# cokwa/bitHTM

Measured on AMD Instinct MI355X. Metric: HTM timesteps/sec (SP + TM, learning on), 65536 cols x 32 cells, higher is better.
Workload: dtype u32 bit-packed / f64 + f32 permanences; 1 GPU; configs[2]: 65536 columns x 32 cells, SP + TM learning on, 1 MI355X; input_dim=1024, column_dim=65536, cell_dim=32, active_columns=1311, patterns=50, pretrain_steps=500, segments=96476, segment_slots=128, hip_graph=True, hip_graph_requested=True, pipelined=True, repetitions=15, streamed_calls=True

## Files before the change

bithtm_amd/build.py:

```python

import json
import os
import re
import subprocess
import sys

HERE = os.path.dirname(os.path.abspath(__file__))
CSRC = os.path.join(HERE, "csrc")
LIB = os.path.join(HERE, "libbithtm_hip.so")
RESOURCES = os.path.join(HERE, "libbithtm_hip.resources.json")
OWN_REPORTS = {"htm_knn.h": os.path.join(HERE, "libbithtm_hip.knn.resources.json")}
SOURCES = ["htm_engine.hip"]
HEADERS = ["htm_dev.h", "htm_sp_kernels.h", "htm_tm_kernels.h", "htm_pipeline.h", "htm_record.h", "htm_reset.h", "htm_decode.h", "htm_stack.h", "htm_forecast.h", "htm_noise.h", "htm_group.h", "htm_tm_feed.h", "htm_sp_run.h", "htm_fork.h", "htm_scalar.h", "htm_live.h", "htm_fields.h", "htm_likelihood.h", "htm_classifier.h", "htm_knn.h", "htm_rng.h", "htm_fexp.h",
           os.path.join("..", "..", "include", "bithtm_hip.h")]
FLAGS = ["--offload-arch=gfx950", "-O3", "-std=c++17", "-fPIC", "-shared", "-ffp-contract=off",
         "-fno-fast-math", "-Wall", "-Wno-unused-result", "-Wno-unused-value",
         "-Rpass-analysis=kernel-resource-usage"]


def _stale():
    if not os.path.exists(LIB) or not all(os.path.exists(r) for r in [RESOURCES] + list(OWN_REPORTS.values())):
        return True
    t = os.path.getmtime(LIB)
    deps = [os.path.join(CSRC, s) for s in SOURCES + HEADERS] + [os.path.abspath(__file__)]
    return any(os.path.getmtime(d) > t for d in deps)


def _kernel_resources(log):
    fields = {"VGPRs": "vgprs", "AGPRs": "agprs", "SGPRs": "sgprs", "ScratchSize [bytes/lane]": "scratch_bytes_per_lane",
              "Occupancy [waves/SIMD]": "occupancy", "LDS Size [bytes/block]": "lds_bytes"}
    out, cur = {}, None
    for line in log.splitlines():
        m = re.search(r"^(?:(\S+?):\d+:\d+: )?remark: +([^:]+): (\S+) \[-Rpass-analysis=kernel-resource-usage\]", line)
        if not m:
            continue
        key, val = m.group(2).strip(), m.group(3)
        if key == "Function Name":
            cur = out.setdefault(os.path.basename(m.group(1) or ""), {}).setdefault(val, {})
        elif cur is not None and key in fields:
            cur[fields[key]] = int(val)
    return out


def _without_remarks(log):
    out, pending, in_remark = [], [], False
    for line in log.splitlines():
        if "kernel-resource-usage" in line:
            pending, in_remark = [], True
        elif line.startswith("In file included from"):
            pending.append(line)
            in_remark = False
        elif in_remark and re.match(r"\s*\d*\s*\|", line):
            continue
        else:
            out += pending + [line]
            pending, in_remark = [], False
    return "\n".join(out)


def build(force=False, verbose=False):
    if not force and not _stale():
        return LIB
    hipcc = os.environ.get("HIPCC", "/opt/rocm/bin/hipcc")
    extra = os.environ.get("BITHTM_EXTRA_FLAGS", "").split()
    cmd = [hipcc] + FLAGS + extra + [os.path.join(CSRC, s) for s in SOURCES] + ["-o", LIB]
    if verbose:
        print(" ".join(cmd), file=sys.stderr)
    r = subprocess.run(cmd, stdout=subprocess.PIPE, stderr=subprocess.STDOUT, text=True)
    if r.returncode != 0:
        raise RuntimeError("hipcc failed:\n" + r.stdout)
    by_header = _kernel_resources(r.stdout)
    for header, path in OWN_REPORTS.items():
        with open(path, "w") as f:
            json.dump(by_header.pop(header, {}), f, indent=0, sort_keys=True)
    with open(RESOURCES, "w") as f:
        json.dump({k: v for kernels in by_header.values() for k, v in kernels.items()}, f, indent=0, sort_keys=True)
    if verbose:
        rest = _without_remarks(r.stdout)
        if rest.strip():
            print(rest, file=sys.stderr)
    return LIB


def kernel_resources(header=None):
    build()
    path = RESOURCES if header is None else OWN_REPORTS[header]
    if not os.path.exists(path):
        return None
    with open(path) as f:
        return json.load(f)


def all_kernel_resources():
    parts = [kernel_resources()] + [kernel_resources(h) for h in OWN_REPORTS]
    return None if any(p is None for p in parts) else {k: v for p in parts for k, v in p.items()}


if __name__ == "__main__":
    print(build(force="--force" in sys.argv, verbose=True))
```

bithtm_amd/csrc/htm_engine.hip:

```cpp

#include <hip/hip_runtime.h>
#include <hip/hip_ext.h>
#include <dlfcn.h>
#include <stdint.h>
#include <stdio.h>
#include <string.h>
#include <algorithm>
#include <cfloat>
#include <climits>
#include <cmath>
#include <chrono>
#include <map>
#include <memory>
#include <mutex>
#include <string>
#include <tuple>
#include <type_traits>
#include <vector>

#include "../../include/bithtm_hip.h"
#include "htm_fexp.h"
#include "htm_rng.h"

#include "htm_dev.h"
#include "htm_sp_kernels.h"
#include "htm_tm_kernels.h"
#include "htm_pipeline.h"
#include "htm_record.h"
#include "htm_reset.h"
#include "htm_decode.h"
#include "htm_stack.h"
#include "htm_forecast.h"
#include "htm_noise.h"
#include "htm_group.h"
#include "htm_tm_feed.h"
#include "htm_sp_run.h"
#include "htm_fork.h"
#include "htm_scalar.h"
#include "htm_live.h"
#include "htm_fields.h"
#include "htm_likelihood.h"
#include "htm_classifier.h"
#include "htm_knn.h"


struct ncclUniqueIdBytes { char internal[128]; };

static thread_local std::string g_create_error;
static int (*g_rccl_destroy)(void *) = nullptr;

struct Knobs {
    int graph_steps, eager_below;
    bool trace;
    uint32_t trace_until;
    int lean, lean2_classify, lean2_order, step_split, fuse_tm, shard_window, step_window, tail_rows, scan_large, scan_large_above, scan_dyn;
    int defer_tail, shared_scan, shared_members;
    int lean_overlap, lean_learn, lean_learn_large, lean_scan, lean_scan_large, scan_blocks, sel_launch_digits;
    int cand_d, cand_pairwise, cls_rows_max, win_offset, cand_zoom, cand_speculate, cand_take_all, poll_delay, cand_others;
};

struct Sizes {
    int G;
    int sp_blocks, sel_blocks, c256_blocks, s1024_blocks, scan_blocks, zero_blocks, cus;
    int lean_learn_blocks, lean_learn_blocks_large, lean_scan_blocks, lean_scan_blocks_large, lean_overlap_blocks, lean2_classify_blocks;
    int lean2_overlap_blocks;
    int lean_resident_large;
    bool emit_fits, emit_fits_open;
    bool emit_fits_lean;
    int sel_passes_fused, sel_passes_full;
};

struct RunModes {
    bool recording, resetting, decoding, feeding;
    bool capturing = false;
    bool operator<(const RunModes &o) const {
        return std::tie(recording, resetting, decoding, feeding, capturing) < std::tie(o.recording, o.resetting, o.decoding, o.feeding, o.capturing);
    }
};

struct RunGraphKey {
    int p; RunModes modes; int learning; bool sp_done, next_sp, next_front, lean; int spec; bool large, emit_fused, wmode;
    int span; const void *bank; int n_inputs;
    auto tie() const { return std::tie(p, modes, learning, sp_done, next_sp, next_front, lean, spec, large, emit_fused, wmode, span, bank, n_inputs); }
    bool operator<(const RunGraphKey &o) const { return tie() < o.tie(); }
};

struct ShardGraphKey {
    int p, learning; bool front_done, front_next; int span, ranks, n_inputs; std::vector<std::tuple<int, bool, bool>> per_rank; const void *bank;
    auto tie() const { return std::tie(p, learning, front_done, front_next, span, ranks, n_inputs, per_rank, bank); }
    bool operator<(const ShardGraphKey &o) const { return tie() < o.tie(); }
};

struct TmRunGraphKey {
    int p; RunModes modes; int learning, spec; bool large; int span; const void *lists; int n_rows, n;
    auto tie() const { return std::tie(p, modes, learning, spec, large, span, lists, n_rows, n); }
    bool operator<(const TmRunGraphKey &o) const { return tie() < o.tie(); }
};

struct SpRunGraphKey {
    int p, learning; bool recording, emit_fused; int wmode, span; const void *bank; int n_inputs;
    auto tie() const { return std::tie(p, learning, recording, emit_fused, wmode, span, bank, n_inputs); }
    bool operator<(const SpRunGraphKey &o) const { return tie() < o.tie(); }
};

struct htm_handle {
    htm_config cfg;
    Dev d;
    Knobs knob;
    Sizes sz;
// ... 322 lines not shown
    if (defer_tail) { h->tail_pending = true; h->tail_p = p; return; }
    if (fuse && (front_wmode >= 0 || n_tail_rows)) {
        const LearnScan ls = learn_scan(h, (size_t)SEL_BINS * 4);
        const int grid = ls.blocks() + (n_tail_rows ? n_tail_rows : h->sz.lean_overlap_blocks);
        const char *name = n_tail_rows ? "tm_learn+tm_scan+sp_learn" : "tm_learn+tm_scan+shard_overlap";
        LAUNCH_ON(h, h->stream, ls.lds, name, kt_learn_scan_tail[ls.slot], grid, 256, d, p, ls.n_learn, ls.n_scan, ls.spec, bank, n_inputs, h->sz.G, front_wmode, n_tail_rows);
        return;
    }
    enqueue_tm_tail(h, p);
    if (front_wmode >= 0)
        LAUNCH(h, "shard_overlap", k_shard_overlap, h->sz.sp_blocks, RB, d, bank, n_inputs, h->sz.G, p, front_wmode, 1);
}

struct StepPlan { bool sp_done, next_sp, next_front; };

static bool can_pipeline(const htm_handle *h) {
    return h->cfg.enable_sp && h->cfg.enable_tm && h->world == 1 && h->emit_fused_open && h->d.sel_passes == 2;
}

static bool can_lean(const htm_handle *h) {
    return h->knob.lean && can_pipeline(h) && bitmap_fits_lds(h->d) && h->sz.emit_fits_lean;
}

static decltype(&k_learn_scan_emit<1, 6>) const kt_lse_large[4] = {k_learn_scan_emit<1, 4, false>, k_learn_scan_emit<2, 4, false>,
                                                                   k_learn_scan_emit<4, 4, false>, k_learn_scan_emit<8, 4, false>};
static decltype(&k_learn_scan_emit<1, 6>) const kt_lse_tab[4] = {k_learn_scan_emit<1, 6, true>, k_learn_scan_emit<2, 6, true>,
                                                                 k_learn_scan_emit<4, 6, true>, k_learn_scan_emit<8, 6, true>};
static decltype(&k_learn_scan_emit<1, 6>) lse_kernel(const Dev &d, int form) {
    return (form == LSE_TAB ? kt_lse_tab : form == LSE_LARGE ? kt_lse_large : kt_lse_plain)[epl_slot(d)];
}

static int lse_form(const htm_handle *h) { return scan_pool_is_large(h) ? LSE_LARGE : lean_tab(h->d) ? LSE_TAB : LSE_PLAIN; }

static void launch_learn_scan_emit(htm_handle *h, int p, int n_emit) {
    Dev &d = h->d;
    const int epl = learn_epl(d);
    const size_t lds = std::max(std::max(learn_lds(epl, 256), lean_scan_lds(d)), sizeof(EmitShared));
    const bool large = scan_pool_is_large(h), dyn = large && h->knob.scan_dyn > 0;
    const int n_learn = dyn ? h->sz.lean_learn_blocks_large : h->sz.lean_learn_blocks;
    int n_scan = large ? h->sz.lean_scan_blocks_large : h->sz.lean_scan_blocks;
    if (dyn) n_scan = std::max(64, h->sz.lean_resident_large - n_emit - n_learn);
    const int grid = n_emit + n_learn + n_scan;
    if (large && !dyn) n_scan = -n_scan;
    const int spec = dyn ? 0 : scan_spec_blocks(h);
    const char *lse_name = large ? "tm_learn+tm_scan_large+sp_emit" : "tm_learn+tm_scan+sp_emit";
    LAUNCH_ON(h, h->stream, lds, lse_name, lse_kernel(d, lse_form(h)), grid, 256, d, p, n_emit, n_learn, n_scan, spec);
}

static int lean2_classify_blocks(const htm_handle *h, int learning) {
    if (!learning) return 0;
    return scan_pool_is_large(h) && !h->knob.lean2_classify ? std::max(h->sz.lean2_classify_blocks, 192) : h->sz.lean2_classify_blocks;
}

static void launch_act_mid_rows(htm_handle *h, const char *name, size_t lds, int p, int learning, const uint32_t *bank, int n_inputs, int n_overlap) {
    Dev &d = h->d;
    const int n_act = act_blocks(d), n_cls = lean2_classify_blocks(h, learning), n_rows = learning ? d.k : 0;
    const int n_duty = n_overlap ? 0 : h->sz.c256_blocks, n_clear = d.WPC * h->sz.c256_blocks;
    LAUNCH_ON(h, h->stream, lds, name, k_act_mid_rows, n_act + 1 + n_cls + n_rows + n_overlap + n_duty + n_clear + h->sz.zero_blocks, 256,
              d, p, d.k, n_act, learning, n_cls, bank, n_inputs, n_rows, h->sz.G, n_overlap, n_duty, n_clear, h->knob.lean2_order);
}

static void enqueue_lean(htm_handle *h, int p, int learning, const uint32_t *bank, int n_inputs, StepPlan plan) {
    Dev &d = h->d;
    if (h->knob.lean == 2) {
        launch_act_mid_rows(h, "tm_activate+tm_mid+sp_learn+sp_overlap", (size_t)SEL_BINS * 4, p, learning, bank, n_inputs,
                            plan.next_sp ? h->sz.lean2_overlap_blocks : 0);
    } else {
        const int n_act = act_blocks(d), n_rows = learning ? d.k : 0;
        const int n_cls = learning ? kClassifyBlocks : 0, n_ov = plan.next_sp ? h->sz.lean_overlap_blocks : 0;
        LAUNCH(h, "tm_activate+sp_learn", k_act_rows, n_act + n_rows + (1 + d.WPC) * h->sz.c256_blocks, 256, d, p, d.k, n_act, bank, n_inputs, n_rows, h->sz.c256_blocks);
        LAUNCH_ON(h, h->stream, (size_t)SEL_BINS * 4, "tm_mid+sp_overlap", k_mid_overlap, 1 + n_cls + n_ov + h->sz.zero_blocks, 256, d, p, d.k, 1, learning, n_cls,
                  bank, n_inputs, h->sz.G, n_ov);
    }
    launch_learn_scan_emit(h, p, plan.next_sp ? h->sz.c256_blocks : 0);
}

static decltype(&k_learn_overlap<1>) const kt_learn_overlap[4] = {k_learn_overlap<1>, k_learn_overlap<2>, k_learn_overlap<4>, k_learn_overlap<8>};
static decltype(&k_scan_sel<true, 1>) const kt_scan_sel[4] = {k_scan_sel<true, 1>, k_scan_sel<false, 1>, k_scan_sel<true, 6>, k_scan_sel<false, 6>};

static void enqueue_pipelined(htm_handle *h, int p, int learning, const uint32_t *bank, int n_inputs, StepPlan plan) {
    Dev &d = h->d;
    const int n_cls = learning ? kClassifyBlocks : 0;
    const int n_emit = plan.next_sp ? h->sz.c256_blocks : 0;
    LAUNCH_ON(h, h->stream, sizeof(EmitShared), "tm_activate+sp_emit", k_open_emit, n_emit + act_blocks(d), 256, d, p, n_emit, d.k);
    const int n_rows = (plan.next_sp && learning) ? d.k : 0, n_duty = plan.next_sp ? h->sz.c256_blocks : 0;
    LAUNCH(h, "tm_mid+sp_learn", k_mid_rows, 1 + n_cls + n_rows + n_duty + h->sz.zero_blocks, 256, d, p, d.k, 1, learning, n_cls, bank, n_inputs, n_rows, 1, n_duty);
    LAUNCH_ON(h, h->stream, std::max(learn_lds(learn_epl(d)), (size_t)SEL_BINS * 4), "tm_learn+sp_overlap", kt_learn_overlap[epl_slot(d)],
              kLearnBlocks + (plan.next_front ? h->sz.sp_blocks : 0), RB, d, p, kLearnBlocks, bank, n_inputs, h->sz.G, p, 2);
    const bool use_lds = bitmap_fits_lds(d), large = scan_pool_is_large(h);
    const int n_sel = plan.next_front ? 64 : 0, n_clear = plan.next_sp ? h->sz.c256_blocks : 0;
    LAUNCH_ON(h, h->stream, std::max(scan_lds(d, use_lds), sizeof(SelShared)), large ? "tm_scan_large+sp_select" : "tm_scan+sp_select",
              kt_scan_sel[scan_slot(large, use_lds)], h->sz.scan_blocks + n_sel + n_clear, 256, d, p, n_sel, n_clear, p, scan_spec_blocks(h));
}

static void enqueue_cold_start(htm_handle *h, const uint32_t *bank, int n_inputs, int learning, StepPlan plan) {
    Dev &d = h->d;
    const int p = (int)(h->step_host & 1);
    if (plan.sp_done || !plan.next_sp) return;
    const int wmode = step_wmode(h);
    if (can_lean(h)) {
        enqueue_sp_front(h, bank, n_inputs, p, wmode);
        enqueue_sp_back(h, bank, n_inputs, p, 1, 0, false, wmode);
        return;
    }
    enqueue_sp_front(h, bank, n_inputs, p, wmode);
    enqueue_sp_back(h, bank, n_inputs, p, 1, EMIT_DUTY | EMIT_CLEAR, learning != 0, wmode);
    LAUNCH(h, "sp_overlap", k_sp_overlap, h->sz.sp_blocks, RB, d, bank, n_inputs, h->sz.G, p, p ^ 1, 1, 0);
    LAUNCH(h, "sp_select", k_sel_pass, h->sz.sel_blocks, RB, d, 1, p ^ 1);
}

static int reset_blocks(const Dev &d) { return std::max(1, std::min(1024, (d.C * d.KP + 255) / 256)); }

static void enqueue_run_reset(htm_handle *h, RunModes m, int p) {
    if (m.resetting) LAUNCH(h, "tm_reset", k_tm_reset, reset_blocks(h->d), 256, h->d, p, h->d_reset, m.recording ? h->d_rec : nullptr, 0u);
}

static void enqueue_rest(htm_handle *h, RunModes m, int p, const uint32_t *bank, int n_inputs, int learning, StepPlan plan) {
    enqueue_run_reset(h, m, p);
    if ((plan.sp_done || plan.next_sp) && can_lean(h)) {
// ... 187 lines not shown
        rc |= dalloc(h, &h->d_cols_stage, k);
    }
    if (h->knob.trace) rc |= dalloc(h, &d.trace, (size_t)8 * 4096 * 2);
    return rc;
}

static const char *env_str(const char *name) { return getenv(name); }
static int env_int(const char *name, int dflt, int lo = INT_MIN, int hi = INT_MAX) {
    const char *e = env_str(name);
    return e ? std::max(lo, std::min(hi, atoi(e))) : dflt;
}
static int env_flag(const char *name, int dflt) {
    const char *e = env_str(name);
    return e ? atoi(e) != 0 : dflt;
}

static Knobs read_knobs() {
    Knobs k;
    k.graph_steps = env_int("BITHTM_GRAPH_STEPS", 16, 1, 256);
    k.eager_below = env_int("BITHTM_EAGER_BELOW", 64, 0);
    k.trace = env_str("BITHTM_TRACE") != nullptr;
    const char *until = env_str("BITHTM_TRACE_UNTIL");
    k.trace_until = until ? (uint32_t)strtoul(until, nullptr, 10) : 0xFFFFFFFFu;
    k.lean = env_int("BITHTM_LEAN", 2, 0, 2);
    k.lean2_classify = env_int("BITHTM_LEAN2_CLASSIFY", 0, 1);
    k.step_split = env_flag("BITHTM_STEP_SPLIT", 1);
    {
        const char *e = env_str("BITHTM_LEAN2_ORDER");
        const int o = e ? (int)strtol(e, nullptr, 16) : 0x0312;
        int seen = 0, pos[4] = {-1, -1, -1, -1};
        for (int i = 0; i < 4; ++i) { const int r = (o >> (4 * (3 - i))) & 15; if (r < 4) { seen |= 1 << r; pos[r] = i; } }
        k.lean2_order = (o >= 0 && o <= 0x3333 && seen == 15 && pos[0] < pos[1]) ? o : 0x0312;
    }
    k.fuse_tm = env_flag("BITHTM_FUSE_TM", 1);
    k.shard_window = env_flag("BITHTM_SHARD_WINDOW", 1);
    k.scan_large = env_int("BITHTM_SCAN_LARGE", -1);
    k.scan_large_above = env_int("BITHTM_SCAN_LARGE_ABOVE", 3 * 1536 * SCAN_SEGS, 0);
    k.step_window = env_flag("BITHTM_STEP_WINDOW", 1);
    k.tail_rows = env_flag("BITHTM_TAIL_ROWS", 1);
    k.scan_dyn = env_flag("BITHTM_SCAN_DYN", 1);
    k.defer_tail = env_flag("BITHTM_DEFER_TAIL", 1);
    k.shared_scan = env_flag("BITHTM_SHARED_SCAN", 0);
    k.shared_members = env_int("BITHTM_SHARED_SCAN_MEMBERS", 0, 0);
    k.lean_overlap = env_int("BITHTM_LEAN_OVERLAP", 0, 1);
    k.lean_learn = env_int("BITHTM_LEAN_LEARN", 0, 1);
    k.lean_learn_large = env_int("BITHTM_LEAN_LEARN_LARGE", 0, 1);
    k.lean_scan = env_int("BITHTM_LEAN_SCAN", 0, 1);
    k.lean_scan_large = env_int("BITHTM_LEAN_SCAN_LARGE", 0, 1);
    k.scan_blocks = env_int("BITHTM_SCAN_BLOCKS", 0, 1);
    k.sel_launch_digits = env_int("BITHTM_SEL_LAUNCH_DIGITS", -1, 0);
    k.cand_d = env_int("BITHTM_CAND_D", CAND_D, 0, CAND_D);
    k.cand_pairwise = env_int("BITHTM_CAND_PAIRWISE", CAND_PAIRWISE, 0);
    k.cls_rows_max = env_int("BITHTM_CLASSIFY_WORDS_ABOVE", -1, 0);
    k.win_offset = env_int("BITHTM_SEL_WINDOW_OFFSET", 0, 0);
    k.cand_zoom = env_int("BITHTM_CAND_ZOOM", -1);
    k.cand_speculate = env_flag("BITHTM_CAND_SPECULATE", 1);
    k.cand_take_all = env_flag("BITHTM_CAND_TAKE_ALL", 1);
    k.poll_delay = env_int("BITHTM_POLL_DELAY", 7, 0, 64);
    k.cand_others = env_int("BITHTM_CAND_OTHERS", CAND_OTHERS, 0, CAND_OTHERS);
    return k;
}

static void size_launches(htm_handle *h) {
    Dev &d = h->d;
    const Knobs &k = h->knob;
    Sizes &z = h->sz;
    z.G = 1;
    while (z.G < d.W4 && z.G < 64) z.G <<= 1;
    const int rows_per_block = (RB / 64) * 4 * (64 / z.G);
    z.sp_blocks = std::max(1, std::min((d.c1 - d.c0 + rows_per_block - 1) / rows_per_block, 256));
    z.sel_blocks = std::max(1, std::min((d.sel_hi - d.sel_lo + RB - 1) / RB, 128));
    z.c256_blocks = (d.sel_hi - d.sel_lo + 255) / 256;
    z.s1024_blocks = std::max(1, (d.Scap + 1023) / 1024);
    z.scan_blocks = std::max(1, std::min((d.Lcap + SCAN_SEGS - 1) / SCAN_SEGS, 2048));
    if (z.scan_blocks > 256) z.scan_blocks = (z.scan_blocks + 255) & ~255;
    z.zero_blocks = std::max(1, std::min((d.Lcap / 128 + 4095) / 4096, 1024));
    z.lean_overlap_blocks = k.lean_overlap ? k.lean_overlap : z.sp_blocks * (RB / 256);
    z.lean2_overlap_blocks = d.planes ? (d.c1 - d.c0 + 255) / 256 : z.lean_overlap_blocks;
    z.lean_learn_blocks = k.lean_learn ? k.lean_learn : 512;
    z.lean_learn_blocks_large = k.lean_learn_large ? k.lean_learn_large : k.lean_learn ? z.lean_learn_blocks : 768;
    z.lean_scan_blocks = k.lean_scan ? k.lean_scan : (z.scan_blocks > 512 ? std::max(256, (z.scan_blocks * 3 / 8 + 255) & ~255) : z.scan_blocks);
    z.lean_scan_blocks_large = k.lean_scan_large ? k.lean_scan_large : k.lean_scan ? z.lean_scan_blocks : z.scan_blocks;
    if (k.scan_blocks) z.scan_blocks = k.scan_blocks;
    hipDeviceProp_t prop;
    const bool have_prop = hipGetDeviceProperties(&prop, h->device) == hipSuccess;
    z.cus = have_prop ? prop.multiProcessorCount : 256;
    int B = 0;
    while ((1ll << B) <= (long long)d.I) ++B;
    const int informative = std::min(64, 64 - (29 - B) - KEY_SHIFT);
    d.sel_passes = std::max(1, std::min(SEL_MAX_PASSES, (informative + SEL_DIGIT - 1) / SEL_DIGIT));
    d.low_zero = 64 - informative;
    int per_cu_emit = 0, per_cu_open = 0;
    if (have_prop && hipOccupancyMaxActiveBlocksPerMultiprocessor(&per_cu_emit, (const void *)k_sp_emit, 256, 0) == hipSuccess &&
        hipOccupancyMaxActiveBlocksPerMultiprocessor(&per_cu_open, (const void *)k_open_emit, 256, sizeof(EmitShared)) == hipSuccess) {
        z.emit_fits = z.c256_blocks <= std::min(1024, per_cu_emit * z.cus);
        z.emit_fits_open = z.emit_fits && z.c256_blocks + act_blocks(d) <= std::min(1024, per_cu_open * z.cus);
        int per_cu_lean = 1 << 30;
        z.lean_resident_large = 1 << 30;
        const size_t lean_lds = std::max(std::max(learn_lds(learn_epl(d), 256), lean_scan_lds(d)), sizeof(EmitShared));
        bool asked = h->cfg.enable_tm && z.emit_fits && lean_lds <= 64 * 1024;
        for (int form = LSE_TAB; asked && form <= LSE_LARGE; ++form) {
            if (form == LSE_TAB && !lean_tab(d)) continue;
            int per_cu = 0;
            asked = hipOccupancyMaxActiveBlocksPerMultiprocessor(&per_cu, (const void *)lse_kernel(d, form), 256, lean_lds) == hipSuccess;
            per_cu_lean = std::min(per_cu_lean, per_cu);
            if (asked && form == LSE_LARGE) z.lean_resident_large = per_cu * z.cus;
        }
        z.emit_fits_lean = asked && z.c256_blocks <= std::min(1024, per_cu_lean * z.cus);
        if (z.lean_resident_large == (1 << 30)) z.lean_resident_large = 4 * z.cus;
    } else {
        (void)hipGetLastError();
        z.emit_fits = z.emit_fits_open = z.emit_fits_lean = false;
        z.lean_resident_large = 1024;
    }
    if (k.lean2_classify) {
        z.lean2_classify_blocks = k.lean2_classify;
    } else {
        int per_cu = 0, resident = 1536;
        if (have_prop && hipOccupancyMaxActiveBlocksPerMultiprocessor(&per_cu, (const void *)k_act_mid_rows, 256, (size_t)SEL_BINS * 4) == hipSuccess)
            resident = per_cu * z.cus;
        else
            (void)hipGetLastError();
        const int others = act_blocks(d) + z.lean_overlap_blocks + d.k + 1;
        const int room = (resident - others) & ~7;
        z.lean2_classify_blocks = room >= 128 ? std::min(kClassifyBlocks, room) : 32;
    }
    z.sel_passes_full = d.sel_passes;
    z.sel_passes_fused = std::min(d.sel_passes, 2);
    if (k.sel_launch_digits >= 0) z.sel_passes_fused = std::max(2, std::min(d.sel_passes, k.sel_launch_digits));
}

extern "C" int htm_create(const htm_config *cfg, htm_handle **out) {
    if (!cfg || !out) return fail_create(nullptr, "htm_create: null argument", HTM_ERR_ARGUMENT);
    if (cfg->struct_bytes != sizeof(htm_config)) return fail_create(nullptr, "htm_create: htm_config size mismatch (ABI)", HTM_ERR_ARGUMENT);
    if (cfg->column_dim < 1 || cfg->active_columns < 1 || cfg->active_columns > cfg->column_dim)
        return fail_create(nullptr, "htm_create: need 1 <= active_columns <= column_dim", HTM_ERR_ARGUMENT);
    if (cfg->enable_sp && cfg->input_dim < 1) return fail_create(nullptr, "htm_create: input_dim < 1", HTM_ERR_ARGUMENT);
    if (cfg->enable_tm) {
        if (cfg->cell_dim < 1 || cfg->cell_dim > 64) return fail_create(nullptr, "htm_create: cell_dim must be in 1..64", HTM_ERR_ARGUMENT);
        if (cfg->segment_slots < 64 || cfg->segment_slots > MAX_SLOTS || cfg->segment_slots % 64)
            return fail_create(nullptr, "htm_create: segment_slots must be a multiple of 64 in 64..512", HTM_ERR_ARGUMENT);
        if (cfg->segment_capacity < 1) return fail_create(nullptr, "htm_create: segment_capacity < 1", HTM_ERR_ARGUMENT);
        if (cfg->segment_sampling_synapses < 1 || cfg->segment_sampling_synapses > 64)
            return fail_create(nullptr, "htm_create: segment_sampling_synapses must be in 1..64", HTM_ERR_ARGUMENT);
        if (cfg->segment_activation_threshold < cfg->segment_matching_threshold)
            return fail_create(nullptr, "htm_create: activation threshold < matching threshold", HTM_ERR_ARGUMENT);
        if ((long long)cfg->column_dim * (cfg->cell_dim > 32 ? 64 : 32) > 0x7FFFFFFFLL) return fail_create(nullptr, "htm_create: column_dim too large", HTM_ERR_ARGUMENT);
    }
    if (!cfg->enable_sp && !cfg->enable_tm) return fail_create(nullptr, "htm_create: nothing enabled", HTM_ERR_ARGUMENT);
    const int world = cfg->shard_world > 1 ? cfg->shard_world : 1;
    if (world > 1) {
        if (!cfg->enable_sp || !cfg->enable_tm) return fail_create(nullptr, "htm_create: a sharded handle needs SP and TM", HTM_ERR_ARGUMENT);
        if (cfg->cell_dim > 32) return fail_create(nullptr, "htm_create: a sharded handle takes cell_dim up to 32 (the exchange record carries one 32-bit word per column)", HTM_ERR_ARGUMENT);
        if (world > 64) return fail_create(nullptr, "htm_create: at most 64 shards", HTM_ERR_ARGUMENT);
        if (cfg->shard_rank < 0 || cfg->shard_rank >= world) return fail_create(nullptr, "htm_create: shard_rank out of range", HTM_ERR_ARGUMENT);
        if (cfg->column_dim % (world * 64)) return fail_create(nullptr, "htm_create: column_dim must be a multiple of 64 * shard_world", HTM_ERR_ARGUMENT);
    }

    htm_handle *h = new htm_handle();
    h->cfg = *cfg;
    h->device = cfg->device;
    h->rank = world > 1 ? cfg->shard_rank : 0;
    h->world = world;
    h->knob = read_knobs();
    hipError_t e = hipSetDevice(cfg->device);
    if (e != hipSuccess) return fail_create(h, std::string("hipSetDevice: ") + hipGetErrorString(e), HTM_ERR_HIP);
    if (cfg->use_caller_stream) {
        h->stream = (hipStream_t)cfg->stream;
    } else {
        e = hipStreamCreateWithFlags(&h->stream, hipStreamNonBlocking);
        if (e != hipSuccess) return fail_create(h, std::string("hipStreamCreate: ") + hipGetErrorString(e), HTM_ERR_HIP);
        h->own_stream = true;
    }
// ... 3724 lines not shown
```

bithtm_amd/csrc/htm_tm_kernels.h:

```cpp
#ifndef BITHTM_HTM_TM_KERNELS_H
#define BITHTM_HTM_TM_KERNELS_H


__global__ __launch_bounds__(256) void k_tm_load_active(Dev d, int p, const int *cols, int n) {
    for (int c = blockIdx.x * 256 + threadIdx.x; c < d.C * d.WPC; c += gridDim.x * 256) {
        d.act[p][c] = 0;
        d.pred[p][c] = 0;
        d.win[p][c] = 0;
        if (c < n) d.active_cols[p][c] = cols[c];
        if (c < d.colwords) d.colbits[p][c] = 0;
    }
}

__global__ __launch_bounds__(256) void k_tm_activate(Dev d, int p, int n_active, int want_winner) {
    role_activate<false, true>(d, p, want_winner, blockIdx.x, n_active);
}

__global__ __launch_bounds__(256) void k_tm_ext_winners(Dev d, int p, const int *cols, const uint32_t *winw, const uint32_t *unacc, int n, int pass) {
    const int i = blockIdx.x * 256 + threadIdx.x;
    if (pass == 0) { for (int c = i; c < d.C * d.WPC; c += gridDim.x * 256) d.win[p][c] = 0; return; }
    if (i < n * d.WPC) {
        const int col = cols[i / d.WPC], wi = col * d.WPC + i % d.WPC;
        if (i % d.WPC == 0) d.active_cols[p][i / d.WPC] = col;
        d.actw_id[i] = wi;
// ... 157 lines not shown
            const u64 m0 = spread32((uint32_t)b0) | (spread32((uint32_t)b1) << 1);
            const u64 m1 = spread32((uint32_t)(b0 >> 32)) | (spread32((uint32_t)(b1 >> 32)) << 1);
            if (lane_id() == 0 && base < d.Ipad) {
                u64 *mw = (u64 *)&mrow[base >> 5];
                mw[0] = m0;
                mw[1] = m1;
            }
            plane_diff_store<16>(d, row, base >> 3, base < d.Ipad, m0, m1, old);
        } else {
            const u64 m0 = spread32((uint32_t)b0) | (spread32((uint32_t)b1) << 1);
            const u64 m1 = spread32((uint32_t)(b0 >> 32)) | (spread32((uint32_t)(b1 >> 32)) << 1);
            plane_diff_store_late<16>(d, mrow, row, i0, m0, m1);
            if (lane_id() == 0 && base < d.Ipad) {
                u64 *mw = (u64 *)&mrow[base >> 5];
                mw[0] = m0;
                mw[1] = m1;
            }
        }
        if (i0 == 0) ROW_STAMP(3); else ROW_STAMP(5);
    }
    if (OWN) {
        __shared__ int s_own[TPR / 64];
        own_cn = (int)wave_sum((uint32_t)own_cn);
        if (lane_id() == 0) s_own[t >> 6] = own_cn;
        __syncthreads();
        if (t == 0) {
            int cn = 0;
#pragma unroll
            for (int wv = 0; wv < TPR / 64; ++wv) cn += s_own[wv];
            const int sp = p ^ 1;
            float dc = duty0 * d.mom;
            dc = dc + d.dinc;
            d.duty[row] = dc;
            d.overlap[sp][row] = cn;
            const float f = htm_exp_f32(d.coef * dc);
            const double bo = (double)f * (double)cn;
            d.boosted[sp][row] = bo;
            const u64 key = select_key(bo);
            d.key[sp][row] = key;
            const uint32_t bin = win_bin(key, wbase);
            if (bin != 0u) {
                atomicAdd(d.hist0 + (size_t)sp * HIST0_PAR + (size_t)(ri & (HIST_REP - 1)) * SEL_BINS + bin, 1u);
                atomicAdd(d.hist0 + (size_t)sp * HIST0_PAR + HIST0_FINE + (size_t)(ri & (COARSE_REP - 1)) * COARSE_STRIDE + (bin >> 6), 1u);
            }
        }
    }
}

template <typename T>
__device__ __forceinline__ T ld_agent(const T *ptr, int same_launch) {
    return same_launch ? __hip_atomic_load(ptr, __ATOMIC_RELAXED, __HIP_MEMORY_SCOPE_AGENT) : *ptr;
}
struct NoWait { __device__ __forceinline__ void operator()() const {} };
template <int BS, typename Wait = NoWait>
__device__ __forceinline__ void role_mid(const Dev &d, int p, int n_active, int want_winner, int learning, int blk, int n_cls, int same_launch = 0,
                                         Wait wait = Wait()) {
    Counters *c = d.ctr;
    __shared__ int s_words[BS];
    __shared__ uint32_t s_bits[BS];
    __shared__ int s_nwords;
    if (blk > 0) {
        if (!learning || !c->has_distal) return;
        const int q = p ^ 1;
        const int n = d.world > 1 ? c->L : c->S;
        bool waited = false;
        auto wait_once = [&]() { if (!waited) { wait(); waited = true; } };
        auto gather = [&](int seg, bool &cand, bool &punish, int &cell) {
            const uint32_t info = d.seg_info[seg];
            cell = d.seg_cell[seg];
            const float jit = d.seg_jit[seg];
            const int cw = cell >> 5, cb = cell & 31, col = cell >> d.LK;
            const bool on_col = (d.colbits[p][col >> 5] >> (col & 31)) & 1u;
            const bool unpred = !((d.pred[q][cw] >> cb) & 1u);
            const bool best = fabsf(jit - __uint_as_float(d.cellmax[q][cell])) < d.eps;
            cand = ((info >> 31) || (unpred && best)) && (on_col || !same_launch);
            punish = d.punish ? (d.punish[cw] >> cb) & 1u : !on_col;
        };
        auto decide = [&](bool cand, int cell) {
            return cand && ((ld_agent(&d.win[p][cell >> 5], same_launch) >> (cell & 31)) & 1u);
        };
        if (n <= (d.cls_rows_max >= 0 ? d.cls_rows_max : (same_launch ? 2 : 8) * n_cls * BS)) {
            for (int i0 = (blk - 1) * BS; i0 < n; i0 += n_cls * BS) {
                const int seg = i0 + (int)threadIdx.x;
                bool cand = false, punish = false;
                int cell = 0;
                if (seg < n && ((d.match_bits[q][seg >> 5] >> (seg & 31)) & 1u)) gather(seg, cand, punish, cell);
                wait_once();
                const bool learn = decide(cand, cell);
                if (learn || punish) d.seg_nsyn[seg] |= (int)SEG_BUSY;
                const u64 ml = __ballot(learn), mp = __ballot(punish);
                const int n_l = __popcll(ml), n_p = __popcll(mp);
                if (n_l + n_p == 0) continue;
                int base = 0;
                if (lane_id() == 0) base = atomicAdd(&c->n_work[p], n_l + n_p);
                base = wave_read(base, 0);
                if (learn) {
                    const int pos = base + __popcll(ml & lanemask_lt());
                    if (pos < d.work_cap) d.work[pos] = (uint32_t)seg; else atomicOr(&c->error, 4);
                }
                if (punish) {
                    const int pos = base + n_l + __popcll(mp & lanemask_lt());
                    if (pos < d.work_cap) d.work[pos] = (uint32_t)seg | 0x80000000u; else atomicOr(&c->error, 4);
                }
            }
            return;
        }
        const int nwords = (n + 31) >> 5;
        const bool by_xcd = n_cls % 8 == 0 && n_cls >= 256;
        const int G8 = by_xcd ? n_cls / 8 : 1, x = (blk - 1) & 7, g = (blk - 1) >> 3;
        const int per_class = ((nwords + 255) >> 8) * 32;
        const int n_turns = by_xcd ? (per_class + G8 - 1) / G8 : (nwords + n_cls - 1) / n_cls;
        for (int t0 = 0; t0 < n_turns; t0 += BS) {
            if (threadIdx.x == 0) s_nwords = 0;
            __syncthreads();
            const int T = t0 + (int)threadIdx.x;
            int w;
            if (by_xcd) {
                const int u = T * G8 + g;
                w = ((x + 8 * (u >> 5)) << 5) + (u & 31);
            } else {
                w = (blk - 1) + n_cls * T;
            }
            const uint32_t word = (T < n_turns && w < nwords) ? d.match_bits[q][w] : 0u;
            if (word) {
                const int slot = atomicAdd(&s_nwords, 1);
                s_words[slot] = w;
                s_bits[slot] = word;
            }
            __syncthreads();
            const int listed = s_nwords;
            for (int i0 = 0; i0 < listed; i0 += BS / 32) {
                const int i = i0 + ((int)threadIdx.x >> 5);
                const bool on = i < listed && ((s_bits[min(i, BS - 1)] >> (threadIdx.x & 31)) & 1u);
                const int seg = on ? s_words[i] * 32 + (int)(threadIdx.x & 31) : 0;
                bool cand = false, punish = false;
                int cell = 0;
                if (on) gather(seg, cand, punish, cell);
                wait_once();
                const bool learn = decide(cand, cell);
                if (learn || punish) d.seg_nsyn[seg] |= (int)SEG_BUSY;
                const u64 ml = __ballot(learn), mp = __ballot(punish);
                const int n_l = __popcll(ml), n_p = __popcll(mp);
                if (n_l + n_p == 0) continue;
                int base = 0;
                if (lane_id() == 0) base = atomicAdd(&c->n_work[p], n_l + n_p);
                base = wave_read(base, 0);
                if (learn) {
                    const int pos = base + __popcll(ml & lanemask_lt());
                    if (pos < d.work_cap) d.work[pos] = (uint32_t)seg; else atomicOr(&c->error, 4);
                }
                if (punish) {
                    const int pos = base + n_l + __popcll(mp & lanemask_lt());
                    if (pos < d.work_cap) d.work[pos] = (uint32_t)seg | 0x80000000u; else atomicOr(&c->error, 4);
                }
            }
        }
        return;
    }
    __shared__ uint32_t s_wave[16];
    __shared__ uint32_t s_cells;
    __shared__ int s_nneed;
    if (threadIdx.x == 0) { s_cells = 0; s_nneed = 0; }
    const int S = c->S, nb = (S + 1023) >> 10;
    const uint32_t recyc_first = (int)threadIdx.x < nb ? (uint32_t)d.recyc_cnt[threadIdx.x] : 0u;
    uint32_t carry_w = 0, carry_u = 0, n_cells = 0;
    constexpr int LPT = 8;
    static_assert(LPT == 8, "the list pass loads 8 entries per thread");
    const int n_slots = n_active * d.WPC;
    const int nb2 = (nb + 1023) >> 10;
    const int cnt2_first = ((int)threadIdx.x < 256 && (int)threadIdx.x < nb2) ? d.recyc_cnt2[threadIdx.x] : 0;
    const int prev_has_winner = c->has_winner[p ^ 1], prev_n_win = c->n_win[p ^ 1];
    const int has_distal_early = same_launch ? c->has_distal : 0;
    wait();
    for (int base = 0; base < n_slots; base += LPT * BS) {
        const int i0 = base + LPT * (int)threadIdx.x;
        uint32_t ww[LPT], uw[LPT];
        int a[LPT];
        uint32_t vsum = 0;
        u64 ac = 0;
        if (i0 < n_slots && same_launch) {
#pragma unroll
            for (int j = 0; j < LPT; j += 2) {
                const u64 av = __hip_atomic_load((const u64 *)(d.actw_id + i0 + j), __ATOMIC_RELAXED, __HIP_MEMORY_SCOPE_AGENT);
                const u64 wv = __hip_atomic_load((const u64 *)(d.winw_idx + i0 + j), __ATOMIC_RELAXED, __HIP_MEMORY_SCOPE_AGENT);
                const u64 uv = __hip_atomic_load((const u64 *)(d.unacc_word + i0 + j), __ATOMIC_RELAXED, __HIP_MEMORY_SCOPE_AGENT);
                a[j] = (int)(uint32_t)av; a[j + 1] = (int)(uint32_t)(av >> 32);
                ww[j] = (uint32_t)wv; ww[j + 1] = (uint32_t)(wv >> 32);
                uw[j] = (uint32_t)uv; uw[j + 1] = (uint32_t)(uv >> 32);
            }
            ac = __hip_atomic_load((const u64 *)(d.actcnt + i0), __ATOMIC_RELAXED, __HIP_MEMORY_SCOPE_AGENT);
        } else if (i0 < n_slots) {
            const int4 a0 = *(const int4 *)(d.actw_id + i0), a1 = *(const int4 *)(d.actw_id + i0 + 4);
            const uint4 w0 = *(const uint4 *)(d.winw_idx + i0), w1 = *(const uint4 *)(d.winw_idx + i0 + 4);
// ... 1042 lines not shown
```

Baseline: 43610 timesteps/s.

## Add handover kernel that builds winner and unaccounted lists in block0 with LDS staging

Adds a specialised variant of the fused activate/mid/rows kernel in which block 0 of the mid role compacts the winner and unaccounted-cell lists itself, then immediately binds recycled and new segments. The unaccounted list is staged in dynamic LDS up to a configurable cap, and scalar pointers are pinned to SGPRs. It also adds an option to prefetch seg_nsyn during gather so the busy mark is a plain store rather than a read-modify-write. The aim is to cut global round-trips and extra kernel phases on the per-step critical path, at the cost of more LDS per block and a possibly lower resident-block count, which the sizing now takes as the minimum over both kernels.

```diff
diff --git a/bithtm_amd/build.py b/bithtm_amd/build.py
--- a/bithtm_amd/build.py
+++ b/bithtm_amd/build.py
@@ -10,8 +10,9 @@
 LIB = os.path.join(HERE, "libbithtm_hip.so")
 RESOURCES = os.path.join(HERE, "libbithtm_hip.resources.json")
 OWN_REPORTS = {"htm_knn.h": os.path.join(HERE, "libbithtm_hip.knn.resources.json")}
+LATER_REPORTS = {"htm_handover.h": os.path.join(HERE, "libbithtm_hip.handover.resources.json")}
 SOURCES = ["htm_engine.hip"]
-HEADERS = ["htm_dev.h", "htm_sp_kernels.h", "htm_tm_kernels.h", "htm_pipeline.h", "htm_record.h", "htm_reset.h", "htm_decode.h", "htm_stack.h", "htm_forecast.h", "htm_noise.h", "htm_group.h", "htm_tm_feed.h", "htm_sp_run.h", "htm_fork.h", "htm_scalar.h", "htm_live.h", "htm_fields.h", "htm_likelihood.h", "htm_classifier.h", "htm_knn.h", "htm_rng.h", "htm_fexp.h",
+HEADERS = ["htm_dev.h", "htm_sp_kernels.h", "htm_tm_kernels.h", "htm_pipeline.h", "htm_record.h", "htm_reset.h", "htm_decode.h", "htm_stack.h", "htm_forecast.h", "htm_noise.h", "htm_group.h", "htm_tm_feed.h", "htm_sp_run.h", "htm_fork.h", "htm_scalar.h", "htm_live.h", "htm_fields.h", "htm_likelihood.h", "htm_classifier.h", "htm_knn.h", "htm_handover.h", "htm_rng.h", "htm_fexp.h",
            os.path.join("..", "..", "include", "bithtm_hip.h")]
 FLAGS = ["--offload-arch=gfx950", "-O3", "-std=c++17", "-fPIC", "-shared", "-ffp-contract=off",
          "-fno-fast-math", "-Wall", "-Wno-unused-result", "-Wno-unused-value",
@@ -19,7 +20,7 @@
 
 
 def _stale():
-    if not os.path.exists(LIB) or not all(os.path.exists(r) for r in [RESOURCES] + list(OWN_REPORTS.values())):
+    if not os.path.exists(LIB) or not all(os.path.exists(r) for r in [RESOURCES] + list(OWN_REPORTS.values()) + list(LATER_REPORTS.values())):
         return True
     t = os.path.getmtime(LIB)
     deps = [os.path.join(CSRC, s) for s in SOURCES + HEADERS] + [os.path.abspath(__file__)]
@@ -70,7 +71,7 @@
     if r.returncode != 0:
         raise RuntimeError("hipcc failed:\n" + r.stdout)
     by_header = _kernel_resources(r.stdout)
-    for header, path in OWN_REPORTS.items():
+    for header, path in list(OWN_REPORTS.items()) + list(LATER_REPORTS.items()):
         with open(path, "w") as f:
             json.dump(by_header.pop(header, {}), f, indent=0, sort_keys=True)
     with open(RESOURCES, "w") as f:
@@ -84,7 +85,7 @@
 
 def kernel_resources(header=None):
     build()
-    path = RESOURCES if header is None else OWN_REPORTS[header]
+    path = RESOURCES if header is None else OWN_REPORTS[header] if header in OWN_REPORTS else LATER_REPORTS[header]
     if not os.path.exists(path):
         return None
     with open(path) as f:
@@ -96,5 +97,10 @@
     return None if any(p is None for p in parts) else {k: v for p in parts for k, v in p.items()}
 
 
+def every_kernel_resources():
+    parts = [all_kernel_resources()] + [kernel_resources(h) for h in LATER_REPORTS]
+    return None if any(p is None for p in parts) else {k: v for p in parts for k, v in p.items()}
+
+
 if __name__ == "__main__":
     print(build(force="--force" in sys.argv, verbose=True))
diff --git a/bithtm_amd/csrc/htm_engine.hip b/bithtm_amd/csrc/htm_engine.hip
--- a/bithtm_amd/csrc/htm_engine.hip
+++ b/bithtm_amd/csrc/htm_engine.hip
@@ -42,6 +42,7 @@
 #include "htm_likelihood.h"
 #include "htm_classifier.h"
 #include "htm_knn.h"
+#include "htm_handover.h"
 
 
 struct ncclUniqueIdBytes { char internal[128]; };
@@ -55,6 +56,7 @@
     uint32_t trace_until;
     int lean, lean2_classify, lean2_order, step_split, fuse_tm, shard_window, step_window, tail_rows, scan_large, scan_large_above, scan_dyn;
     int defer_tail, shared_scan, shared_members;
+    int handover_cap;
     int lean_overlap, lean_learn, lean_learn_large, lean_scan, lean_scan_large, scan_blocks, sel_launch_digits;
     int cand_d, cand_pairwise, cls_rows_max, win_offset, cand_zoom, cand_speculate, cand_take_all, poll_delay, cand_others;
 };
@@ -483,19 +485,25 @@
     return scan_pool_is_large(h) && !h->knob.lean2_classify ? std::max(h->sz.lean2_classify_blocks, 192) : h->sz.lean2_classify_blocks;
 }
 
-static void launch_act_mid_rows(htm_handle *h, const char *name, size_t lds, int p, int learning, const uint32_t *bank, int n_inputs, int n_overlap) {
+static void launch_act_mid_rows(htm_handle *h, const char *name, size_t lds, int p, int learning, const uint32_t *bank, int n_inputs, int n_overlap,
+                                bool handover = false) {
     Dev &d = h->d;
     const int n_act = act_blocks(d), n_cls = lean2_classify_blocks(h, learning), n_rows = learning ? d.k : 0;
     const int n_duty = n_overlap ? 0 : h->sz.c256_blocks, n_clear = d.WPC * h->sz.c256_blocks;
-    LAUNCH_ON(h, h->stream, lds, name, k_act_mid_rows, n_act + 1 + n_cls + n_rows + n_overlap + n_duty + n_clear + h->sz.zero_blocks, 256,
-              d, p, d.k, n_act, learning, n_cls, bank, n_inputs, n_rows, h->sz.G, n_overlap, n_duty, n_clear, h->knob.lean2_order);
+    const int grid = n_act + 1 + n_cls + n_rows + n_overlap + n_duty + n_clear + h->sz.zero_blocks;
+    if (handover)
+        LAUNCH_ON(h, h->stream, std::max(lds, (size_t)SEL_BINS * 4), name, k_first_handover, grid, 256,
+                  d, p, d.k, n_act, learning, n_cls, bank, n_inputs, n_rows, h->sz.G, n_overlap, n_duty, n_clear, h->knob.lean2_order, h->knob.handover_cap);
+    else
+        LAUNCH_ON(h, h->stream, lds, name, k_act_mid_rows, grid, 256,
+                  d, p, d.k, n_act, learning, n_cls, bank, n_inputs, n_rows, h->sz.G, n_overlap, n_duty, n_clear, h->knob.lean2_order);
 }
 
 static void enqueue_lean(htm_handle *h, int p, int learning, const uint32_t *bank, int n_inputs, StepPlan plan) {
     Dev &d = h->d;
     if (h->knob.lean == 2) {
         launch_act_mid_rows(h, "tm_activate+tm_mid+sp_learn+sp_overlap", (size_t)SEL_BINS * 4, p, learning, bank, n_inputs,
-                            plan.next_sp ? h->sz.lean2_overlap_blocks : 0);
+                            plan.next_sp ? h->sz.lean2_overlap_blocks : 0, true);
     } else {
         const int n_act = act_blocks(d), n_rows = learning ? d.k : 0;
         const int n_cls = learning ? kClassifyBlocks : 0, n_ov = plan.next_sp ? h->sz.lean_overlap_blocks : 0;
@@ -789,6 +797,7 @@
     k.cand_d = env_int("BITHTM_CAND_D", CAND_D, 0, CAND_D);
     k.cand_pairwise = env_int("BITHTM_CAND_PAIRWISE", CAND_PAIRWISE, 0);
     k.cls_rows_max = env_int("BITHTM_CLASSIFY_WORDS_ABOVE", -1, 0);
+    k.handover_cap = env_int("BITHTM_HANDOVER_LDS_CAP", HANDOVER_LIST_MAX, 0, HANDOVER_LIST_MAX);
     k.win_offset = env_int("BITHTM_SEL_WINDOW_OFFSET", 0, 0);
     k.cand_zoom = env_int("BITHTM_CAND_ZOOM", -1);
     k.cand_speculate = env_flag("BITHTM_CAND_SPECULATE", 1);
@@ -854,8 +863,10 @@
         z.lean2_classify_blocks = k.lean2_classify;
     } else {
         int per_cu = 0, resident = 1536;
-        if (have_prop && hipOccupancyMaxActiveBlocksPerMultiprocessor(&per_cu, (const void *)k_act_mid_rows, 256, (size_t)SEL_BINS * 4) == hipSuccess)
-            resident = per_cu * z.cus;
+        int per_cu_run = 0;
+        if (have_prop && hipOccupancyMaxActiveBlocksPerMultiprocessor(&per_cu, (const void *)k_act_mid_rows, 256, (size_t)SEL_BINS * 4) == hipSuccess &&
+            hipOccupancyMaxActiveBlocksPerMultiprocessor(&per_cu_run, (const void *)k_first_handover, 256, (size_t)SEL_BINS * 4) == hipSuccess)
+            resident = std::min(per_cu, per_cu_run) * z.cus;
         else
             (void)hipGetLastError();
         const int others = act_blocks(d) + z.lean_overlap_blocks + d.k + 1;
diff --git a/bithtm_amd/csrc/htm_handover.h b/bithtm_amd/csrc/htm_handover.h
--- /dev/null
+++ b/bithtm_amd/csrc/htm_handover.h
@@ -0,0 +1,262 @@
+#ifndef BITHTM_HANDOVER_H
+#define BITHTM_HANDOVER_H
+
+#define HANDOVER_NEED 128
+#define HANDOVER_LIST_MAX (SEL_BINS - 2 * HANDOVER_NEED - 256)
+static_assert(HANDOVER_LIST_MAX >= 1024, "the dynamic LDS of the launch (SEL_BINS words) holds the list, the needed blocks and the counts");
+
+#ifdef BITHTM_HANDOVER_STAMPS
+#define HSTAMP(i, v) do { if (d.trace && threadIdx.x == 0 && d.ctr->step[p] < d.trace_until) d.trace[(size_t)(3 + 4 * p) * 8192 + (i)] = (v); } while (0)
+#else
+#define HSTAMP(i, v) do { } while (0)
+#endif
+
+template <typename Wait>
+__device__ __forceinline__ void role_handover_block0(const Dev &d, int p, int n_active, int learning, int list_cap, uint32_t *dyn, Wait wait) {
+    constexpr int BS = 256, LPT = 8;
+    Counters *c = d.ctr;
+    int *s_un = (int *)dyn, *s_need = (int *)dyn + HANDOVER_LIST_MAX, *s_cnt2 = s_need + 2 * HANDOVER_NEED;
+    __shared__ uint32_t s_wave[16];
+    __shared__ uint32_t s_cells;
+    __shared__ int s_nneed;
+    if (threadIdx.x == 0) { s_cells = 0; s_nneed = 0; }
+    const int S = c->S, nb = (S + 1023) >> 10;
+    const uint32_t recyc_first = (int)threadIdx.x < nb ? (uint32_t)d.recyc_cnt[threadIdx.x] : 0u;
+    int n_slots = n_active * d.WPC;
+    const int nb2 = (nb + 1023) >> 10;
+    const int cnt2_first = (int)threadIdx.x < nb2 ? d.recyc_cnt2[threadIdx.x] : 0;
+    const int prev_has_winner = c->has_winner[p ^ 1], prev_n_win = c->n_win[p ^ 1];
+    const int has_distal = c->has_distal;
+    typedef __attribute__((address_space(1))) int gint;
+    typedef __attribute__((address_space(1))) const u64 gu64c;
+    gu64c *actw_id = (gu64c *)d.actw_id, *winw_idx = (gu64c *)d.winw_idx, *unacc_word = (gu64c *)d.unacc_word, *actcnt = (gu64c *)d.actcnt;
+    gint *winners = (gint *)d.winners[p], *unacc_list = (gint *)d.unacc_list, *seg_nsyn = (gint *)d.seg_nsyn, *seg_cell = (gint *)d.seg_cell;
+    typedef __attribute__((address_space(1))) Counters gctr;
+    gctr *ctr = (gctr *)c;
+    int match_thr = d.match_thr, Scap = d.Scap;
+#ifndef BITHTM_HANDOVER_NO_PIN
+    asm volatile("" : "+s"(actw_id), "+s"(winw_idx), "+s"(unacc_word), "+s"(actcnt), "+s"(winners), "+s"(unacc_list), "+s"(seg_nsyn), "+s"(seg_cell),
+                      "+s"(match_thr), "+s"(Scap), "+s"(ctr), "+s"(n_slots));
+#endif
+    c = (Counters *)ctr;
+    HSTAMP(0, wall_clock64());
+    wait();
+    HSTAMP(1, wall_clock64());
+    uint32_t carry_w = 0, carry_u = 0, n_cells = 0;
+    uint32_t ww[LPT];
+    int a[LPT];
+    uint32_t run_w = 0;
+    for (int base = 0; base < n_slots; base += LPT * BS) {
+        const int i0 = base + LPT * (int)threadIdx.x;
+        uint32_t uw[LPT];
+        uint32_t vsum = 0;
+        u64 ac = 0;
+        if (i0 < n_slots) {
+#pragma unroll
+            for (int j = 0; j < LPT; j += 2) {
+                const u64 av = __hip_atomic_load(actw_id + ((i0 + j) >> 1), __ATOMIC_RELAXED, __HIP_MEMORY_SCOPE_AGENT);
+                const u64 wv = __hip_atomic_load(winw_idx + ((i0 + j) >> 1), __ATOMIC_RELAXED, __HIP_MEMORY_SCOPE_AGENT);
+                const u64 uv = __hip_atomic_load(unacc_word + ((i0 + j) >> 1), __ATOMIC_RELAXED, __HIP_MEMORY_SCOPE_AGENT);
+                a[j] = (int)(uint32_t)av; a[j + 1] = (int)(uint32_t)(av >> 32);
+                ww[j] = (uint32_t)wv; ww[j + 1] = (uint32_t)(wv >> 32);
+                uw[j] = (uint32_t)uv; uw[j + 1] = (uint32_t)(uv >> 32);
+            }
+            ac = __hip_atomic_load(actcnt + (i0 >> 3), __ATOMIC_RELAXED, __HIP_MEMORY_SCOPE_AGENT);
+#pragma unroll
+            for (int j = 0; j < LPT; ++j) {
+                const bool ok = i0 + j < n_slots;
+                if (!ok) { ww[j] = 0; uw[j] = 0; }
+                n_cells += ok ? (uint32_t)((ac >> (8 * j)) & 0xFFu) : 0u;
+            }
+        } else {
+#pragma unroll
+            for (int j = 0; j < LPT; ++j) { a[j] = 0; ww[j] = 0; uw[j] = 0; }
+        }
+#pragma unroll
+        for (int j = 0; j < LPT; ++j) vsum += (uint32_t)__popc(ww[j]) | ((uint32_t)__popc(uw[j]) << 16);
+        uint32_t total;
+        const uint32_t run = block_excl_scan<BS, true>(vsum, s_wave, total);
+        run_w = carry_w + (run & 0xFFFFu);
+        int pu = (int)(carry_u + (run >> 16));
+#pragma unroll
+        for (int j = 0; j < LPT; ++j) {
+            uint32_t u1 = uw[j];
+            while (u1) {
+                const int b = __ffs(u1) - 1;
+                u1 &= u1 - 1;
+                if (pu < list_cap) s_un[pu] = a[j] * 32 + b; else unacc_list[pu] = a[j] * 32 + b;
+                ++pu;
+            }
+        }
+        if (base + LPT * BS < n_slots) {
+            int pw = (int)run_w;
+#pragma unroll
+            for (int j = 0; j < LPT; ++j) {
+                uint32_t w1 = ww[j];
+                while (w1) { const int b = __ffs(w1) - 1; w1 &= w1 - 1; winners[pw++] = a[j] * 32 + b; }
+            }
+        }
+        carry_w += total & 0xFFFFu;
+        carry_u += total >> 16;
+    }
+    n_cells = wave_sum(n_cells);
+    if (lane_id() == 0) atomicAdd(&s_cells, n_cells);
+    const int n_un = (learning && has_distal) ? (int)carry_u : 0;
+    auto finish = [&](int n_r, int n_new, bool bound) {
+        int pw = (int)run_w;
+#pragma unroll
+        for (int j = 0; j < LPT; ++j) {
+            uint32_t w1 = ww[j];
+            while (w1) { const int b = __ffs(w1) - 1; w1 &= w1 - 1; winners[pw++] = a[j] * 32 + b; }
+        }
+        for (int i = threadIdx.x; i < min((int)carry_u, list_cap); i += BS) unacc_list[i] = s_un[i];
+        HSTAMP(8, wall_clock64());
+        if (threadIdx.x == 0) {
+            c->n_win[p] = (int)carry_w;
+            c->has_winner[p] = 1;
+            c->n_un = n_un;
+            c->n_active_cells = (int)s_cells;
+            c->n_bind[p] = bound ? n_r + n_new : 0;
+            if (bound) {
+                c->n_recycled = n_r;
+                c->n_new = n_new;
+                c->S_old = S;
+                c->S = S + n_new;
+            }
+        }
+    };
+    lds_barrier();
+    HSTAMP(2, wall_clock64());
+    HSTAMP(6, (unsigned long long)n_un);
+    if (n_un == 0) { finish(0, 0, false); return; }
+    uint32_t carry = 0;
+    for (int r0 = 0; r0 < nb2 && carry < (uint32_t)n_un; r0 += 256) {
+        lds_barrier();
+        s_cnt2[threadIdx.x] = r0 == 0 ? cnt2_first : (r0 + (int)threadIdx.x < nb2 ? d.recyc_cnt2[r0 + threadIdx.x] : 0);
+        lds_barrier();
+        for (int r = r0; r < min(r0 + 256, nb2) && carry < (uint32_t)n_un; ++r) {
+            if (s_cnt2[r - r0] == 0) continue;
+            for (int base = r << 10; base < min(nb, (r + 1) << 10); base += BS) {
+                const int b = base + threadIdx.x;
+                const uint32_t v = base == 0 ? recyc_first : ((b < nb && b < ((r + 1) << 10)) ? (uint32_t)d.recyc_cnt[b] : 0u);
+                uint32_t total;
+                const uint32_t ex = block_excl_scan<BS, true>(v, s_wave, total);
+                if (v > 0 && carry + ex < (uint32_t)n_un) {
+                    const int slot = atomicAdd(&s_nneed, 1);
+                    if (slot < HANDOVER_NEED) {
+                        s_need[2 * slot] = b;
+                        s_need[2 * slot + 1] = (int)(carry + ex);
+                    } else {
+                        d.recyc_need[2 * slot] = b;
+                        d.recyc_need[2 * slot + 1] = (int)(carry + ex);
+                    }
+                }
+                carry += total;
+                if (carry >= (uint32_t)n_un) break;
+            }
+        }
+    }
+    lds_barrier();
+    const int n_need = s_nneed;
+    HSTAMP(3, wall_clock64());
+    HSTAMP(7, (unsigned long long)n_need);
+    if (n_un > list_cap || n_need > HANDOVER_NEED) __syncthreads();
+    const int n_r = min(n_un, (int)carry);
+    int n_new = n_un - n_r;
+    if (S + n_new > Scap) {
+        if (threadIdx.x == 0) atomicOr(&c->error, 1);
+        n_new = max(Scap - S, 0);
+    }
+    auto listed = [&](int i) { return i < list_cap ? s_un[i] : unacc_list[i]; };
+    const int wbase = d.work_cap - (n_r + n_new);
+    const int n_w = prev_has_winner ? prev_n_win : -1;
+    const int grown = n_w > 0 ? min(d.sample, n_w) : 0;
+    for (int i = 0; i < n_need; ++i) {
+        const int b = i < HANDOVER_NEED ? s_need[2 * i] : d.recyc_need[2 * i], off = i < HANDOVER_NEED ? s_need[2 * i + 1] : d.recyc_need[2 * i + 1];
+        constexpr int IPT = 1024 / BS;
+        int owner[IPT];
+        uint32_t fl[IPT], cnt = 0;
+#pragma unroll
+        for (int j = 0; j < IPT; ++j) {
+            const int seg = b * 1024 + (int)threadIdx.x * IPT + j, at = min(seg, Scap - 1);
+            const bool dead = seg_nsyn[at] < match_thr;
+            owner[j] = seg_cell[at];
+            fl[j] = (seg < S && dead) ? 1u : 0u;
+            cnt += fl[j];
+        }
+        uint32_t total;
+        int rank = off + (int)block_excl_scan<BS, true>(cnt, s_wave, total);
+#pragma unroll
+        for (int j = 0; j < IPT; ++j) {
+            const int seg = b * 1024 + (int)threadIdx.x * IPT + j;
+            if (fl[j] && rank < n_r) {
+                const int cell = listed(rank), pos = wbase + rank;
+                atomicSub(&d.segcount[owner[j]], 1);
+                seg_cell[seg] = cell;
+                seg_nsyn[seg] = (int)SEG_BUSY;
+                atomicAdd(&d.segcount[cell], 1);
+                if (pos < d.work_cap) d.work[pos] = (uint32_t)seg; else atomicOr(&c->error, 4);
+            }
+            rank += (int)fl[j];
+        }
+        if (threadIdx.x == 0 && grown >= d.match_thr) recyc_add(d, b, -max(0, min((int)total, n_r - off)));
+    }
+    HSTAMP(4, wall_clock64());
+    for (int i = threadIdx.x; i < n_new; i += BS) tm_bind_segment(d, S + i, listed(n_r + i), false, wbase + n_r + i);
+    if (n_new > 0 && grown < d.match_thr)
+        for (int b = (S >> 10) + (int)threadIdx.x; b <= (S + n_new - 1) >> 10; b += BS)
+            recyc_add(d, b, min(S + n_new, (b + 1) << 10) - max(S, b << 10));
+    finish(n_r, n_new, true);
+    HSTAMP(5, wall_clock64());
+}
+
+#ifndef BITHTM_HANDOVER_PRE_NSYN
+#define BITHTM_HANDOVER_PRE_NSYN true
+#endif
+
+__global__ __launch_bounds__(256, BITHTM_LEAN2_WAVES) void k_first_handover(Dev d, int p, int n_active, int n_act_blocks, int learning, int n_cls,
+                                                        const uint32_t *__restrict__ bank, int n_inputs, int n_rows, int G, int n_overlap_blocks,
+                                                        int n_duty_blocks, int n_clear_blocks, int order, int list_cap) {
+    TraceScope ts(d, 0 + 4 * p);
+    int b = blockIdx.x;
+    int role = 4;
+#pragma unroll
+    for (int i = 3; i >= 0 && role == 4; --i) {
+        const int r = (order >> (4 * i)) & 15;
+        const int n = r == 0 ? n_act_blocks : r == 1 ? 1 + n_cls : r == 2 ? n_rows : n_overlap_blocks;
+        if (b < n) role = r; else b -= n;
+    }
+    if (role == 0) {
+        role_activate<true>(d, p, 1, b, n_active);
+        fan_signal(d, p, b);
+        return;
+    }
+    if (role == 1) {
+        auto wait = [&]() { fan_wait(d, p, (uint32_t)n_act_blocks); };
+        if (b == 0) role_handover_block0(d, p, n_active, learning, list_cap, (uint32_t *)dyn_lds, wait);
+        else { __builtin_assume(b > 0); role_mid<256, decltype(wait), BITHTM_HANDOVER_PRE_NSYN>(d, p, n_active, 1, learning, b, n_cls, 1, wait); }
+        return;
+    }
+    if (role == 2) {
+        if (n_overlap_blocks > 0) role_sp_row<256, true>(d, p, bank, n_inputs, 0, b, threadIdx.x);
+        else role_sp_row<256>(d, p, bank, n_inputs, 0, b, threadIdx.x);
+        return;
+    }
+    if (role == 3) {
+        if (d.planes) role_overlap_planes(d, bank, n_inputs, p, p ^ 1, 1, b, n_overlap_blocks, (uint32_t *)dyn_lds, n_rows > 0 ? 2 : 1);
+        else role_overlap<256>(d, bank, n_inputs, G, p, p ^ 1, 1, b, n_overlap_blocks, (uint32_t *)dyn_lds, 1, n_rows > 0 ? 2 : 1);
+        return;
+    }
+    if (b < n_duty_blocks) {
+        role_duty(d, p, b, 0, d.C);
+        return;
+    }
+    b -= n_duty_blocks;
+    if (b < n_clear_blocks) {
+        role_clear_dense(d, p, b, n_clear_blocks);
+        return;
+    }
+    role_zero_match(d, p, b - n_clear_blocks, (int)gridDim.x - n_act_blocks - 1 - n_cls - n_rows - n_overlap_blocks - n_duty_blocks - n_clear_blocks, d.ctr->S);
+}
+
+#endif
diff --git a/bithtm_amd/csrc/htm_tm_kernels.h b/bithtm_amd/csrc/htm_tm_kernels.h
--- a/bithtm_amd/csrc/htm_tm_kernels.h
+++ b/bithtm_amd/csrc/htm_tm_kernels.h
@@ -233,7 +233,7 @@
     return same_launch ? __hip_atomic_load(ptr, __ATOMIC_RELAXED, __HIP_MEMORY_SCOPE_AGENT) : *ptr;
 }
 struct NoWait { __device__ __forceinline__ void operator()() const {} };
-template <int BS, typename Wait = NoWait>
+template <int BS, typename Wait = NoWait, bool PRE_NSYN = false>
 __device__ __forceinline__ void role_mid(const Dev &d, int p, int n_active, int want_winner, int learning, int blk, int n_cls, int same_launch = 0,
                                          Wait wait = Wait()) {
     Counters *c = d.ctr;
@@ -246,7 +246,8 @@
         const int n = d.world > 1 ? c->L : c->S;
         bool waited = false;
         auto wait_once = [&]() { if (!waited) { wait(); waited = true; } };
-        auto gather = [&](int seg, bool &cand, bool &punish, int &cell) {
+        auto gather = [&](int seg, bool &cand, bool &punish, int &cell, int &nsyn) {
+            if (PRE_NSYN) nsyn = d.seg_nsyn[seg];
             const uint32_t info = d.seg_info[seg];
             cell = d.seg_cell[seg];
             const float jit = d.seg_jit[seg];
@@ -260,15 +261,18 @@
         auto decide = [&](bool cand, int cell) {
             return cand && ((ld_agent(&d.win[p][cell >> 5], same_launch) >> (cell & 31)) & 1u);
         };
+        auto mark_busy = [&](int seg, int nsyn) {
+            if (PRE_NSYN) d.seg_nsyn[seg] = nsyn | (int)SEG_BUSY; else d.seg_nsyn[seg] |= (int)SEG_BUSY;
+        };
         if (n <= (d.cls_rows_max >= 0 ? d.cls_rows_max : (same_launch ? 2 : 8) * n_cls * BS)) {
             for (int i0 = (blk - 1) * BS; i0 < n; i0 += n_cls * BS) {
                 const int seg = i0 + (int)threadIdx.x;
                 bool cand = false, punish = false;
-                int cell = 0;
-                if (seg < n && ((d.match_bits[q][seg >> 5] >> (seg & 31)) & 1u)) gather(seg, cand, punish, cell);
+                int cell = 0, nsyn = 0;
+                if (seg < n && ((d.match_bits[q][seg >> 5] >> (seg & 31)) & 1u)) gather(seg, cand, punish, cell, nsyn);
                 wait_once();
                 const bool learn = decide(cand, cell);
-                if (learn || punish) d.seg_nsyn[seg] |= (int)SEG_BUSY;
+                if (learn || punish) mark_busy(seg, nsyn);
                 const u64 ml = __ballot(learn), mp = __ballot(punish);
                 const int n_l = __popcll(ml), n_p = __popcll(mp);
                 if (n_l + n_p == 0) continue;
@@ -315,11 +319,11 @@
                 const bool on = i < listed && ((s_bits[min(i, BS - 1)] >> (threadIdx.x & 31)) & 1u);
                 const int seg = on ? s_words[i] * 32 + (int)(threadIdx.x & 31) : 0;
                 bool cand = false, punish = false;
-                int cell = 0;
-                if (on) gather(seg, cand, punish, cell);
+                int cell = 0, nsyn = 0;
+                if (on) gather(seg, cand, punish, cell, nsyn);
                 wait_once();
                 const bool learn = decide(cand, cell);
-                if (learn || punish) d.seg_nsyn[seg] |= (int)SEG_BUSY;
+                if (learn || punish) mark_busy(seg, nsyn);
                 const u64 ml = __ballot(learn), mp = __ballot(punish);
                 const int n_l = __popcll(ml), n_p = __popcll(mp);
                 if (n_l + n_p == 0) continue;
```

Measured after the change: 44550 timesteps/s (median of 6 runs). 2.2% higher.
